# kevaday/alphazero-general

Measured on AMD Instinct MI355X. Metric: mcts_node_expansions_per_sec, higher is better.
Workload: dtype f32 tree / f16 net; 1 GPU; connect4 self-play, 2048 games/GPU x 100 sims/move, fp16 ResNet 128ch x 8, random-init, noise+temp on; games_per_gpu=2048, sims_per_move=100, hipgraph_rounds=True, stream_pipelines=1, fused_search_launch=True, mfma_tower=True, ranks=1

## Files before the change

alphazero_general_amd/build.py:

```python
import os
import subprocess
import sys

HERE = os.path.dirname(os.path.abspath(__file__))
SRC = os.path.join(HERE, 'csrc', 'azg_engine.hip')
DEPS = [os.path.join(HERE, 'csrc', f) for f in sorted(os.listdir(os.path.join(HERE, 'csrc')))] + \
       [os.path.join(os.path.dirname(HERE), 'include', 'azg.h')]
OUT = os.path.join(HERE, 'lib', 'libazg_hip.so')
FLAGS = ['--offload-arch=gfx950', '-O3', '-std=c++17', '-ffp-contract=off', '-fPIC', '-shared']
VARIANTS = {
    'product': ('libazg_hip.so', []),
    'debug': ('libazg_debug.so', ['-DAZG_DEBUG_BOUNDS']),
    'tuning': ('libazg_tuning.so', ['-DAZG_TUNING']),
    'timing-tree': ('libazg_timing.so', ['-DAZG_TREE_TIMING']),
    'timing-tower': ('libazg_timing.so', ['-DAZG_TOWER_TIMING']),
    'timing-w1': ('libazg_timing_w1.so', ['-DAZG_TOWER_TIMING', '-DAZG_PHASE_TID=64', '-DAZG_TUNING']),
    'timing-w1-overlap': ('libazg_timing_w1o.so', ['-DAZG_TOWER_TIMING', '-DAZG_PHASE_TID=64', '-DAZG_OVL_NW=2', '-DHEADS_A_RING=1', '-DAZG_TUNING']),
    'ring1': ('libazg_ring1.so', ['-DHEADS_A_RING=1', '-DAZG_TUNING']),
    'overlap': ('libazg_overlap.so', ['-DAZG_OVL_NW=2', '-DHEADS_A_RING=1', '-DAZG_TUNING']),
    'headline1': ('libazg_headline1.so', ['-DAZG_HEADLINE_ONE_WG']),
}


def hipcc():
    for c in (os.environ.get('HIPCC'), '/opt/rocm/bin/hipcc', 'hipcc'):
        if c and (os.path.isabs(c) and os.path.exists(c) or not os.path.isabs(c)):
            return c
    return 'hipcc'


def source_sha(variant='product'):
    import hashlib
    h = hashlib.sha256()
    for f in DEPS:
# ... 34 lines not shown
```

alphazero_general_amd/csrc/azg_conv.h:

```cpp
#pragma once
#include <hip/hip_runtime.h>
#include <stdint.h>
#include <type_traits>

namespace azg {

typedef _Float16 half8 __attribute__((ext_vector_type(8)));
typedef _Float16 half4 __attribute__((ext_vector_type(4)));
typedef float floatx4 __attribute__((ext_vector_type(4)));

struct TowerParams {
    const void *x;
    const void *w;
    const float *bias;
    const float *pre_scale;
    const float *pre_shift;
    void *y;
    int boards, nblocks;
    const void *head_w;
    const float *head_b;
    float *policy, *value;
    int A, NV;
    unsigned long long *dbg;
    const void *head1_w;
    const float *head1_b;
// ... 535 lines not shown
    if constexpr (__is_same(SEARCH, NoSearch)) return 0; else return sa.ev.gcount[GC_ERROR];
}
template <class SEARCH, class = void> struct WideGameOf { using type = C4; };
template <class SEARCH> struct WideGameOf<SEARCH, std::void_t<typename SEARCH::Game>> { using type = typename SEARCH::Game; };
#ifdef AZG_HEADLINE_ONE_WG
#define AZG_SEARCH_MIN_BLOCKS 1
#else
#define AZG_SEARCH_MIN_BLOCKS 2
#endif
template <class SEARCH> constexpr int tower_min_blocks() { if constexpr (__is_same(SEARCH, NoSearch)) return 2; else { if constexpr (SEARCH::WIDE) return SEARCH::MIN_BLOCKS; else return AZG_SEARCH_MIN_BLOCKS; } }

template <int H, int W, int C> constexpr bool tower_khalf_order() { return ((H == 7 && W == 7) || (H == 8 && W == 8)) && C == 64; }
template <int C, int BOARDS> constexpr int tower_layer_param_bytes(int nblocks) { return ((2 * nblocks + 1) * C * 4 + 2 * nblocks * C * 2 + C * 4 + 15) / 16 * 16; }
template <int C, int BOARDS, bool SOLO = false> constexpr int tower_param_bytes(int nblocks) {
    return BOARDS == 1 ? tower_layer_param_bytes<C, BOARDS>(nblocks) + (C / 32) * 2 * 1024 + 128 : SOLO ? tower_layer_param_bytes<C, BOARDS>(nblocks) : 0;
}
template <int H, int W, int BOARDS, int C, int PSPLIT = 1, class SEARCH = NoSearch, int KSPLIT = 1>
__global__ __launch_bounds__(C * 2 * PSPLIT * KSPLIT, tower_min_blocks<SEARCH>()) void k_tower2(TowerParams Pin, const int16_t *pixmap, SEARCH sa) {
    using GEO = TowerGeom<H, W, BOARDS, C>;
    constexpr bool IS_SEARCH = !__is_same(SEARCH, NoSearch);
    constexpr bool IS_WIDE = []() { if constexpr (IS_SEARCH) return SEARCH::WIDE; else return false; }();
    static_assert(!IS_SEARCH || IS_WIDE || (PSPLIT == 1 && C == 128 && BOARDS <= C / 32), "search mode: one wave per game, fused heads");
    constexpr bool IS_ARENA = []() { if constexpr (IS_SEARCH) { if constexpr (!SEARCH::WIDE) return SEARCH::ARENA; } return false; }();
    static_assert(!IS_ARENA || BOARDS == 1, "arena search: one game (one mover, one model) per workgroup");
    constexpr bool IS_WARENA = []() { if constexpr (IS_SEARCH) { if constexpr (SEARCH::WIDE) return SEARCH::ARENA; } return false; }();
    static_assert(!IS_WARENA || BOARDS == 1, "wide arena search: one game (one mover, one model) per workgroup");
    static_assert(!IS_WIDE || (C / 32) * PSPLIT * KSPLIT >= BOARDS, "wide search mode: at least one wavefront per game");
    constexpr bool SOLO = IS_WIDE && wide_solo<C, PSPLIT, KSPLIT, BOARDS>();
    constexpr bool EXACT = []() { if constexpr (IS_WIDE) return SEARCH::EXACT; else return false; }();
    constexpr bool HSTREAM = HeadsStreamedOf<SEARCH, H * W, C>::value;
// ... 124 lines not shown
        if constexpr (IS_SEARCH) nsims = sa.sims + (IS_WIDE ? 1 : 0);
        [[maybe_unused]] const int sc_off = PARAM_OFF + (2 * P.nblocks + 1) * C * 4, sh_off = sc_off + P.nblocks * C * 2;
        [[maybe_unused]] const int h1_off = PARAM_OFF + tower_layer_param_bytes<C, BOARDS>(P.nblocks);
        if (PLDS && !raw) {
            float *pb_ = reinterpret_cast<float *>(smem + PARAM_OFF);
            _Float16 *psc_ = reinterpret_cast<_Float16 *>(smem + sc_off), *psh_ = reinterpret_cast<_Float16 *>(smem + sh_off);
            for (int c = tid; c < (2 * P.nblocks + 1) * C; c += NT) pb_[c] = P.bias[c];
            for (int c = tid; c < P.nblocks * C; c += NT) { psc_[c] = (_Float16)P.pre_scale[c]; psh_[c] = (_Float16)P.pre_shift[c]; }
            if (PLDS_H1 && P.head_w == nullptr && P.head1_w != nullptr) {
                uint4 *h1_ = reinterpret_cast<uint4 *>(smem + h1_off);
                for (int c = tid; c < KS * 2 * 64; c += NT) h1_[c] = reinterpret_cast<const uint4 *>(P.head1_w)[c];
                if (tid < 32) reinterpret_cast<float *>(smem + h1_off + KS * 2 * 1024)[tid] = P.head1_b[tid];
            }
        }
        [[maybe_unused]] bool lds_live = false;
        for (int sim = 0; sim < nsims; sim++) {
        int lane_sim = lane_k;
        if constexpr (IS_WIDE) asm volatile("" : "+v"(lane_sim));
        const int lane = lane_sim, tid = wave * 64 + lane, g = lane >> 4, i16 = lane & 15;
#ifdef AZG_TOWER_TIMING
        unsigned long long wt_[6] = {0, 0, 0, 0, 0, 0};
#define AZG_WPHASE(i) do { if (IS_WIDE) wt_[i] = __builtin_amdgcn_s_memtime(); } while (0)
#else
#define AZG_WPHASE(i) do { } while (0)
#endif
        AZG_WPHASE(0);
        if constexpr (IS_WIDE) {
            using G = typename SEARCH::Game;
            using WS = WideScratch<G, HW, SOLO>;
            static_assert(G::CELLS == HW, "game / tower geometry mismatch");
// ... 208 lines not shown
                } else {
                    char *row = img + GEO::qrow(bd * HW + lane) * RS;
                    const uint4 z = make_uint4(0, 0, 0, 0);
                    *reinterpret_cast<uint4 *>(row) = z; *reinterpret_cast<uint4 *>(row + 16) = z;
                    *reinterpret_cast<uint4 *>(row + 32) = z; *reinterpret_cast<uint4 *>(row + 48) = z;
                }
            }
            if (sim == sa.sims) break;
            AZG_WPHASE(1);
            if (raw) { __syncthreads(); continue; }
        } else if constexpr (IS_SEARCH) {
            using G = typename SEARCH::Game;
            static_assert(G::CELLS == HW && G::A < 8, "search mode needs a game whose tree functions use no LDS scratch");
            if ((sim & 15) == 0) {
                int *flag = reinterpret_cast<int *>(img + SCRATCH_PV + 512);
                if (tid == 0) *flag = sa.ev.gcount[GC_ERROR];
                __syncthreads();
                const int err = *flag;
                __syncthreads();
                if (tid == 0) *flag = 0;
                if (err) break;
            }
            int slot = tile * BOARDS + wave;
            asm volatile("" : "+v"(slot));
            slot = __builtin_amdgcn_readfirstlane(slot);
            if (wave >= BOARDS) {
            } else if (slot < sa.ev.B) {
                select_slot<G>(sa.ev, slot, lane, nullptr, [&](const typename G::S &st, int ln) {
                    if (ln < HW) {
                        char *row = img + GEO::qrow(wave * HW + ln) * RS;
                        *reinterpret_cast<half8 *>(row) = G::obs8(st, ln);
                        const uint4 z = make_uint4(0, 0, 0, 0);
                        *reinterpret_cast<uint4 *>(row + 16) = z; *reinterpret_cast<uint4 *>(row + 32) = z; *reinterpret_cast<uint4 *>(row + 48) = z;
                    }
                });
            } else if (lane < HW) {
                char *row = img + GEO::qrow(wave * HW + lane) * RS;
                const uint4 z = make_uint4(0, 0, 0, 0);
                *reinterpret_cast<uint4 *>(row) = z; *reinterpret_cast<uint4 *>(row + 16) = z;
                *reinterpret_cast<uint4 *>(row + 32) = z; *reinterpret_cast<uint4 *>(row + 48) = z;
            }
        } else {
            const uint4 *xg = reinterpret_cast<const uint4 *>(P.x) + (size_t)row0;
            for (int c = tid; c < ROWS * 4; c += NT) {
                const int p = c >> 2, chunk = c & 3;
                uint4 v = make_uint4(0, 0, 0, 0);
                if (chunk == 0 && p < rows_here) v = xg[p];
                *reinterpret_cast<uint4 *>(img + GEO::qrow(p) * RS + chunk * 16) = v;
            }
        }
#ifdef AZG_TOWER_TIMING
        if (P.dbg && tid == 0) P.dbg[1024 + blockIdx.x * 2] = __builtin_amdgcn_s_memtime();
#endif
        const half8 *wt = wm0;
#pragma unroll
        for (int j = 0; j < WR - 1; j++) { const half8 *f = stream_frag<GEO, KSPLIT>(wl, wm0, j); a[j][0] = f[0]; a[j][1] = f[64]; }
#ifdef AZG_TOWER_TIMING
        asm volatile("s_waitcnt vmcnt(0)");
        if (P.dbg && tid == 0) P.dbg[1024 + blockIdx.x * 2 + 1] = __builtin_amdgcn_s_memtime();
#endif
        __syncthreads();
#ifdef AZG_TOWER_TIMING
#define AZG_STAMP2(i) do { if (P.dbg && blockIdx.x == 0 && tile == 0 && lane == 0) P.dbg[(layer * 4 + wave) * 5 + (i)] = __builtin_amdgcn_s_memtime(); } while (0)
#define AZG_WGSTAMP(i) do { if (P.dbg && tid == 0) P.dbg[2048 + (size_t)blockIdx.x * 8 + (i)] = __builtin_amdgcn_s_memtime(); } while (0)
#else
#define AZG_STAMP2(i) do { } while (0)
#define AZG_WGSTAMP(i) do { } while (0)
#endif
        AZG_WGSTAMP(4);
        [[maybe_unused]] floatx4 bnext[2];
        if constexpr (PLDS) {
#pragma unroll
            for (int m = 0; m < 2; m++) bnext[m] = *reinterpret_cast<const floatx4 *>(smem + PARAM_OFF + ((2 * cg + m) * 16 + g * 4) * 4);
        }
        for (int layer = 0; layer <= 2 * P.nblocks; layer++) {
            AZG_STAMP2(0);
            if ((layer ^ slot_role) & 1) __builtin_amdgcn_s_setprio(2); else __builtin_amdgcn_s_setprio(0);
            const float *bias = P.bias + (size_t)layer * C;
            const bool is_s = (layer & 1) == 0;
            const int nb = layer >> 1;
            const bool has_next = nb < P.nblocks;
            const half2v zero2 = {(_Float16)0.f, (_Float16)0.f};
#pragma unroll
            for (int m = 0; m < 2; m++) {
// ... 109 lines not shown
                        } else {
                            *reinterpret_cast<uint4 *>(img + off) = *reinterpret_cast<uint4 *>(v);
                        }
                    }
                }
            }
            if constexpr (PLDS) {
#pragma unroll
                for (int m = 0; m < 2; m++) bnext[m] = *reinterpret_cast<const floatx4 *>(smem + PARAM_OFF + ((layer + 1) * C + (2 * cg + m) * 16 + g * 4) * 4);
            }
            AZG_STAMP2(3);
            __syncthreads();
            AZG_STAMP2(4);
        }
        AZG_WGSTAMP(5);
        AZG_WPHASE(2);
        if (P.head_w == nullptr && P.head1_w != nullptr) {
            [[maybe_unused]] _Float16 *feat_lds = nullptr;
            if constexpr (IS_WIDE) feat_lds = reinterpret_cast<_Float16 *>(smem + TILE + WideScratch<typename SEARCH::Game, HW, SOLO>::FEAT);
            using HGame = typename std::conditional<IS_WIDE, typename WideGameOf<SEARCH>::type, C4>::type;
            [[maybe_unused]] HeadsFirst<HGame, HW, HSTREAM ? HEADS_STREAM_RING : WideScratch<HGame, HW>::FK / 32> hfirst;
            constexpr bool HEADS_EARLY = EXACT && BOARDS == 1;
            if constexpr (OVL) {
                if (wave >= 1 && wave <= OVL_NW) heads_full_prefetch<typename SEARCH::Game, HW, OVL_NW, true>(hfs, wave - 1, lane, hfirst);
                if (IS_WIDE && tid == 0 && (sim & 15) == 15) {
                    using WLE = WideLds<typename WideGameOf<SEARCH>::type, HW, BOARDS, SOLO, HSTREAM>;
                    *reinterpret_cast<int *>(smem + TILE + WLE::ERR) = sa_error_word(sa);
                }
            } else
            if constexpr (HSTREAM) { static_assert(HEADS_EARLY && !OVL, "streamed heads: the one-game exact tile"); heads_stream_prefetch<typename SEARCH::Game, HW, NT / 64>(hfs, wave, lane, hfirst); } else
// ... 108 lines not shown
                            if (!bvalid || p >= HW) bf[j][ks] = zero8;
                        }
                    }
                }
                __builtin_amdgcn_sched_barrier(0);
#pragma unroll
                for (int j = 0; j < JB; j++)
                    if (j0 + j < NPW) {
#pragma unroll
                        for (int ks = 0; ks < 4; ks++) hacc4[ks] = __builtin_amdgcn_mfma_f32_16x16x32_f16(af[j][ks], bf[j][ks], hacc4[ks], 0, 0, 0);
                    }
                __builtin_amdgcn_sched_barrier(0);
            }
            const floatx4 hacc = (hacc4[0] + hacc4[1]) + (hacc4[2] + hacc4[3]);
            AZG_WGSTAMP(6);
            __syncthreads();
            float *red = reinterpret_cast<float *>(img);
            if (wave < 4) {
#pragma unroll
                for (int r = 0; r < 4; r++) red[(wave * 16 + g * 4 + r) * 16 + i16] = hacc[r];
            }
            __syncthreads();
            const int nb_here = min(BOARDS, P.boards - tile * BOARDS);
            if (tid < 64) {
                const int bd = tid >> 4, o = tid & 15, A = P.A, NV = P.NV;
                const int bc = bd < BOARDS ? bd : 0;
                const float lgt = ((red[(0 * 16 + o) * 16 + bc] + red[(1 * 16 + o) * 16 + bc]) + (red[(2 * 16 + o) * 16 + bc] + red[(3 * 16 + o) * 16 + bc]))
                                  + P.head_b[o];
                const bool isp = o < A, isv = o >= A && o < A + NV;
                float mp = isp ? lgt : -INFINITY, mv = isv ? lgt : -INFINITY;
#pragma unroll
                for (int d = 8; d; d >>= 1) { mp = fmaxf(mp, __shfl_xor(mp, d, 16)); mv = fmaxf(mv, __shfl_xor(mv, d, 16)); }
                const float e = isp ? __expf(lgt - mp) : isv ? __expf(lgt - mv) : 0.f;
                float sp = isp ? e : 0.f, sv = isv ? e : 0.f;
#pragma unroll
                for (int d = 8; d; d >>= 1) { sp += __shfl_xor(sp, d, 16); sv += __shfl_xor(sv, d, 16); }
                if constexpr (IS_SEARCH) {
                    reinterpret_cast<float *>(img + SCRATCH_PV)[bd * 16 + o] = isp ? e / sp : e / sv;
                } else if (bd < nb_here) {
                    if (isp) P.policy[(size_t)(tile * BOARDS + bd) * A + o] = e / sp;
                    if (isv) P.value[(size_t)(tile * BOARDS + bd) * NV + (o - A)] = e / sv;
                }
            }
            if constexpr (IS_SEARCH) {
                using G = typename SEARCH::Game;
                __syncthreads();
                int slot = tile * BOARDS + wave;
                asm volatile("" : "+v"(slot));
                slot = __builtin_amdgcn_readfirstlane(slot);
                const float *pv = reinterpret_cast<const float *>(img + SCRATCH_PV) + wave * 16;
                if (wave < BOARDS && slot < sa.ev.B) backup_slot<G>(sa.ev, slot, lane, pv, pv + P.A, nullptr, nullptr);
            }
            AZG_WGSTAMP(7);
            __syncthreads();
            if (tid < 256) reinterpret_cast<uint4 *>(img)[tid] = make_uint4(0, 0, 0, 0);
            if constexpr (IS_SEARCH) { if (tid < 16) reinterpret_cast<uint4 *>(img + SCRATCH_PV)[tid] = make_uint4(0, 0, 0, 0); }
        }
        if constexpr (!OVL) __syncthreads();
        }
        if constexpr (IS_WIDE) {
            using G = typename SEARCH::Game;
            using WS = WideScratch<G, HW, SOLO>;
            __syncthreads();
            const int bd = wave % BOARDS, role = wave / BOARDS, slot = tile * BOARDS + bd;
            const int tree = IS_WARENA ? slot * sa.ev.T + (reinterpret_cast<const int *>(smem + TILE + WideLds<G, HW, BOARDS, SOLO, HSTREAM>::ERR)[1] & 15) : slot;
            if (lds_live && role == 0 && slot < sa.ev.B) {
                const char *ws = smem + TILE + bd * WS::BYTES;
                if (lane < 4) reinterpret_cast<uint4 *>(sa.ev.hdr + tree)[lane] = reinterpret_cast<const uint4 *>(ws + WS::HDR)[lane];
                static_assert(sizeof(TreeHdr) == 4 * sizeof(uint4) && sizeof(azg_state) % 16 == 0 && sizeof(PathEnt) == sizeof(uint4),
                              "the LDS mirror moves the header, the root state and the path as whole 16-byte chunks");
                if constexpr (!SOLO) {
                    const int depth = *reinterpret_cast<const int *>(ws + WS::HDR + offsetof(TreeHdr, depth));
                    for (int j = lane; j < depth && j < sa.ev.maxd; j += 64)
                        reinterpret_cast<uint4 *>(sa.ev.path + (size_t)tree * sa.ev.maxd)[j] = reinterpret_cast<const uint4 *>(ws + WS::PATH)[j];
// ... 17 lines not shown
```

alphazero_general_amd/csrc/azg_engine.hip:

```cpp
#include <hip/hip_runtime.h>
#include <hip/hip_ext.h>
#include <cstdio>
#include <cstdlib>
#include <cstring>
#include <map>
#include <mutex>
#include <string>
#include <vector>
#include "azg_kernels.h"
#include "azg_conv.h"

using namespace azg;

static thread_local std::string g_err;
static int fail(int code, const std::string &msg) { g_err = msg; return code; }
#define HIPCHK(x) do { hipError_t _e = (x); if (_e != hipSuccess) return fail(AZG_E_HIP, std::string(#x) + ": " + hipGetErrorString(_e)); } while (0)

struct EvPair { hipEvent_t a, b; bool ext; };

static thread_local EvPair *g_kev = nullptr;
#define AZG_LAUNCH(kernel, grid, block, lds, stream, ...) do { \
    if (g_kev) { hipExtLaunchKernelGGL(kernel, grid, block, lds, stream, g_kev->a, g_kev->b, 0, __VA_ARGS__); g_kev = nullptr; } \
    else hipLaunchKernelGGL(kernel, grid, block, lds, stream, __VA_ARGS__); } while (0)

// ... 778 lines not shown
    if (LDS_BYTES > (size_t)d_lds[dev]) return fail(AZG_E_INVALID_ARG, "this tower does not fit the LDS of its tile (too many residual blocks)");
    if (occ) {
        int n = 0;
        HIPCHK(hipOccupancyMaxActiveBlocksPerMultiprocessor(&n, reinterpret_cast<const void *>(&k_tower2<H, W, BOARDS, C, PSPLIT, SEARCH, KSPLIT>),
                                                            C * 2 * PSPLIT * KSPLIT, LDS_BYTES));
        *occ = n > 0 ? n : 1;
    }
    if (init_only) return AZG_OK;
    HIPCHK(hipDeviceGetAttribute(&cus, hipDeviceAttributeMultiprocessorCount, dev));
    const int ntiles = (P.boards + BOARDS - 1) / BOARDS + (P.rows_per_model ? P.nmodels - 1 : 0);
    {
        const int per_cu = (int)((size_t)d_lds[dev] / LDS_BYTES) > 0 ? (int)((size_t)d_lds[dev] / LDS_BYTES) : 1;
        const int grid = IS_SEARCH || ntiles < per_cu * cus ? ntiles : per_cu * cus;
#ifdef AZG_TOWER_TIMING
        static unsigned long long *dbg = nullptr; static int calls = 0;
        if (!dbg) { HIPCHK(hipMalloc((void **)&dbg, (2048 + 4096 * 8) * 8)); HIPCHK(hipMemset(dbg, 0, (2048 + 4096 * 8) * 8)); }
        TowerParams Q = P; Q.dbg = dbg;
        AZG_LAUNCH((k_tower2<H, W, BOARDS, C, PSPLIT, SEARCH, KSPLIT>), dim3(grid), dim3(C * 2 * PSPLIT * KSPLIT), LDS_BYTES, s, Q, (const int16_t *)d_map[dev], sa);
        if constexpr (IS_SEARCH) if constexpr (SEARCH::WIDE) {
            static unsigned long long w[512 * 4];
            HIPCHK(hipStreamSynchronize(s)); HIPCHK(hipMemcpy(w, dbg + 2048 + 4096 * 4, sizeof(unsigned long long) * 4 * (grid < 512 ? grid : 512), hipMemcpyDeviceToHost));
            double ph[4] = {0, 0, 0, 0}; const int nb = grid < 512 ? grid : 512;
            for (int b = 0; b < nb; b++) for (int i = 0; i < 4; i++) ph[i] += (double)w[b * 4 + i];
            const double n = (double)nb * (sa.sims > 8 ? sa.sims - 8 : 1);
            fprintf(stderr, "wide search, cycles per simulation (mean over %d workgroups): tree %.0f tower %.0f headconv %.0f heads %.0f\n", nb, ph[0] / n, ph[1] / n, ph[2] / n, ph[3] / n);
            HIPCHK(hipMemset(dbg + 2048 + 4096 * 4, 0, sizeof(unsigned long long) * 4 * 512));
            static unsigned long long hw_[512 * 8];
            HIPCHK(hipMemcpy(hw_, dbg + 2048 + 4096 * 5, sizeof(unsigned long long) * 8 * nb, hipMemcpyDeviceToHost));
            double hp[5] = {0, 0, 0, 0, 0}, hn = 0;
            for (int b = 0; b < nb; b++) { for (int i = 0; i < 5; i++) hp[i] += (double)hw_[b * 8 + i]; hn += (double)hw_[b * 8 + 5]; }
            if (hn > 0) fprintf(stderr, "  helper wavefront (cycles per simulation with a policy backup): header %.0f masks %.0f logits %.0f softmax %.0f priors %.0f\n",
                                hp[0] / hn, hp[1] / hn, hp[2] / hn, hp[3] / hn, hp[4] / hn);
            HIPCHK(hipMemset(dbg + 2048 + 4096 * 5, 0, sizeof(unsigned long long) * 8 * 512));
            {
                unsigned long long h[64 * 4 * 5];
                HIPCHK(hipMemcpy(h, dbg, sizeof(h), hipMemcpyDeviceToHost));
                for (int l = 0; l <= 2 * P.nblocks; l++) for (int w = 0; w < C / 32 * PSPLIT * KSPLIT && w < 4; w++) {
                    unsigned long long *t = h + (l * 4 + w) * 5;
                    fprintf(stderr, "  layer %2d wave %d: main %6llu wait %6llu epi %6llu bar %6llu | start %llu\n", l, w, t[1] - t[0], t[2] - t[1], t[3] - t[2], t[4] - t[3], t[0] - h[0]);
                }
            }
            calls = 100;
        }
        if (++calls == 8) {
            unsigned long long h[64 * 4 * 5];
            HIPCHK(hipStreamSynchronize(s)); HIPCHK(hipMemcpy(h, dbg, sizeof(h), hipMemcpyDeviceToHost));
            for (int l = 0; l <= 2 * P.nblocks; l++) for (int w = 0; w < C / 32; w++) {
                unsigned long long *t = h + (l * 4 + w) * 5;
                fprintf(stderr, "layer %2d wave %d: main %6llu wait %6llu epi %6llu bar %6llu | start %llu\n", l, w, t[1] - t[0], t[2] - t[1], t[3] - t[2], t[4] - t[3], t[0] - h[0]);
            }
            static unsigned long long w[4096 * 8];
            HIPCHK(hipMemcpy(w, dbg + 2048, sizeof(unsigned long long) * 8 * grid, hipMemcpyDeviceToHost));
            unsigned long long x2[1024];
            HIPCHK(hipMemcpy(x2, dbg + 1024, sizeof(x2), hipMemcpyDeviceToHost));
            for (int b = 0; b < grid && b < 512; b++) fprintf(stderr, "wgx %4d xload+store %llu weights %llu\n", b, x2[b * 2] - w[b * 8], x2[b * 2 + 1] - x2[b * 2]);
            for (int b = 0; b < grid; b++) fprintf(stderr, "wg %4d xcc %llu hwid %08llx start %llu end %llu | prologue %llu layers %llu headmm %llu softmax %llu tail %llu\n", b, w[b * 8 + 3] & 15, w[b * 8 + 2], w[b * 8], w[b * 8 + 1],
                                                   w[b * 8 + 4] - w[b * 8], w[b * 8 + 5] - w[b * 8 + 4], w[b * 8 + 6] - w[b * 8 + 5], w[b * 8 + 7] - w[b * 8 + 6], w[b * 8 + 1] - w[b * 8 + 7]);
        }
// ... 195 lines not shown
    return r;
}

extern "C" int azg_search_f16(azg_engine *e, void *stream, const void *w, const float *bias, const float *pre_scale, const float *pre_shift,
                              int nblocks, const void *head_w, const float *head_b, int sims) {
    if (!e || !w || !bias || !head_w || !head_b || nblocks < 0 || sims < 0) return fail(AZG_E_INVALID_ARG, "null or out-of-range argument");
    if (nblocks > 0 && (!pre_scale || !pre_shift)) return fail(AZG_E_INVALID_ARG, "pre_scale/pre_shift required");
    if (e->cfg.game != AZG_GAME_CONNECT4 || e->v.arena)
        return fail(AZG_E_UNSUPPORTED, "the fused search kernel is built for connect4 self-play with a 128-channel tower (use azg_select / network / azg_backup)");
    const int A = e->gi.action_size, NV = e->gi.num_players + 1;
    TowerParams P{nullptr, w, bias, pre_scale, pre_shift, nullptr, e->v.B, nblocks, head_w, head_b, nullptr, nullptr, A, NV, nullptr, nullptr, nullptr, nullptr, 0, nullptr, 0, {}};
    SearchArgs<C4> sa{e->v, sims};
    EvPair ep; const bool prof = sims > 0 && netprof_begin((hipStream_t)stream, ep);
    int r, cus = 1;
    r = device_cus(&cus); if (r != AZG_OK) { g_kev = nullptr; return r; }
    if (2 * e->v.B <= 5 * cus) r = launch_tower<C4::H, C4::W, 1, 128, 1, SearchArgs<C4>>((hipStream_t)stream, P, sa, sims == 0);
    else if (e->v.B <= 5 * cus) r = launch_tower<C4::H, C4::W, 2, 128, 1, SearchArgs<C4>>((hipStream_t)stream, P, sa, sims == 0);
    else r = launch_tower<C4::H, C4::W, 4, 128, 1, SearchArgs<C4>>((hipStream_t)stream, P, sa, sims == 0);
    netprof_end((hipStream_t)stream, 2, prof, ep);
    return r;
}

extern "C" int azg_search_arena_f16(azg_engine *e, void *stream, int nmodels, const void *const *w, const float *const *bias, const float *const *pre_scale,
                                    const float *const *pre_shift, int nblocks, const void *const *head_w, const float *const *head_b,
                                    const int32_t *p2i_host, const uint32_t *seat_of_slot, int sims) {
    if (!e || !w || !bias || !head_w || !head_b || nblocks < 0 || sims < 0 || (!p2i_host && !seat_of_slot)) return fail(AZG_E_INVALID_ARG, "null or out-of-range argument");
    if (e->cfg.game != AZG_GAME_CONNECT4 || !e->v.arena)
        return fail(AZG_E_UNSUPPORTED, "the persistent arena launch is built for connect4 arena engines with 128-channel towers (use azg_select / network / azg_backup)");
    if (nmodels < 1 || nmodels > 4 || nmodels < e->gi.num_players) return fail(AZG_E_UNSUPPORTED, "one model per player, at most 4");
    for (int m = 0; m < nmodels; m++)
        if (!w[m] || !bias[m] || !head_w[m] || !head_b[m] || (nblocks > 0 && (!pre_scale || !pre_shift || !pre_scale[m] || !pre_shift[m]))) return fail(AZG_E_INVALID_ARG, "null model parameter");
    const int A = e->gi.action_size, NV = e->gi.num_players + 1;
// ... 397 lines not shown
```

alphazero_general_amd/csrc/azg_kernels.h:

```cpp
#pragma once
#include "azg_games.h"

namespace azg {

struct NodeR {
    int n; float q, p, v; int fc; int a, nchild, player, e;
};
AZG_DEV void unpack(const uint4 &lo, const uint4 &hi, NodeR &r) {
    r.n = (int)lo.x; r.q = __uint_as_float(lo.y); r.p = __uint_as_float(lo.z); r.v = __uint_as_float(lo.w);
    r.fc = (int)hi.x; r.a = hi.y & 0xFFFF; r.nchild = hi.y >> 16; r.player = hi.z & 0xFF; r.e = (hi.z >> 8) & 0xFF;
}
AZG_DEV uint4 pack_hi(int fc, int a, int nchild, int player, int e) {
    return make_uint4((unsigned)fc, (unsigned)(a & 0xFFFF) | ((unsigned)nchild << 16), (unsigned)player | ((unsigned)e << 8), 0u);
}
AZG_DEV void load_node(const Node *p, uint4 &lo, uint4 &hi) {
    const uint4 *q = reinterpret_cast<const uint4 *>(p);
    lo = q[0]; hi = q[1];
}
AZG_DEV void raise_error(const View &ev, int code) { atomicCAS(&ev.gcount[GC_ERROR], 0, code); }
#ifdef AZG_DEBUG_BOUNDS
AZG_DEV bool bounds_fail(const View &ev, int site) { raise_error(ev, AZG_E_INTERNAL); atomicCAS(&ev.gcount[GC_BOUNDS_SITE], 0, site); return false; }
#define AZG_BOUNDS_OK(ev, site, cond) ((cond) ? true : bounds_fail(ev, site))
#else
#define AZG_BOUNDS_OK(ev, site, cond) true
// ... 323 lines not shown
        for (int a = 0; a < A; a++) {
            uint64_t bal = __ballot(ca[0] == a);
            if (bal) s += rl(cp[0], __ffsll((unsigned long long)bal) - 1);
        }
        return s;
    } else {
        if (first) { for (int a = lane; a < A; a += 64) m_lds[a] = 0.f; }
        wave_sync();
#pragma unroll
        for (int c = 0; c < NC; c++) if (ca[c] >= 0) m_lds[ca[c]] = cp[c];
        wave_sync();
        return np_sum_static<A>(m_lds, scr, lane);
    }
}

template <class G, int NC>
AZG_DEV void leaf_policy(const View &ev, int slot, Node *nodes, int fc, int k, bool at_root, const float *pi, float *m_lds, float *scr, int lane) {
    int ca[NC]; float cp[NC];
#pragma unroll
    for (int c = 0; c < NC; c++) {
        int i = c * 64 + lane;
        ca[c] = i < k ? (int)nodes[fc + i].a : -1;
        cp[c] = i < k ? pi[ca[c]] : 0.f;
    }
    const float s = masked_sum<G, NC>(ev, ca, cp, m_lds, scr, lane, true);
    if (!(s > 0.f) && lane == 0) raise_error(ev, AZG_E_FLOATING_POINT);
#pragma unroll
    for (int c = 0; c < NC; c++) cp[c] = cp[c] / s;
    if (at_root && ev.add_temp) {
        const double ex = 1.0 / (double)ev.root_temp;
#pragma unroll
        for (int c = 0; c < NC; c++) cp[c] = np_pow_f32(cp[c], ex);
        const float s2 = masked_sum<G, NC>(ev, ca, cp, m_lds, scr, lane, false);
#pragma unroll
        for (int c = 0; c < NC; c++) cp[c] = cp[c] / s2;
    }
    if (at_root && ev.add_noise) {
        const uint64_t ctr = ev.tape_ctr[slot];
// ... 18 lines not shown
            const double inv = 1.0 / acc;
#pragma unroll
            for (int c = 0; c < NC; c++) nzv[c] = (float)(g[c] * inv);
        }
#pragma unroll
        for (int c = 0; c < NC; c++) {
            const float nz = nzv[c];
            cp[c] = (float)(((double)cp[c] * (1.0 - (double)ev.noise_frac)) + (double)(ev.noise_frac * nz));
        }
        if (lane == 0) ev.tape_ctr[slot] = ctr + 1;
    }
#pragma unroll
    for (int c = 0; c < NC; c++) { int i = c * 64 + lane; if (i < k) nodes[fc + i].p = cp[c]; }
}

template <class G>
AZG_DEV void backup_policy(const View &ev, int slot, const HdrR &hr, Node *nodes, const float *pi, float *m_lds, float *scr, int lane) {
    constexpr int NCH = (G::MAXK + 63) / 64;
    if (hr.leaf_e || hr.leaf_fc < 0) return;
    const int k = hr.leaf_k, fc = hr.leaf_fc;
    if (!AZG_BLOCK_OK(ev, 4, fc, k, hr.alloc)) return;
    const bool at_root = hr.leaf == LEAF_IS_ROOT;
    if constexpr (NCH > 1) {
        if (k > 64) leaf_policy<G, NCH>(ev, slot, nodes, fc, k, at_root, pi, m_lds, scr, lane);
        else leaf_policy<G, 1>(ev, slot, nodes, fc, k, at_root, pi, m_lds, scr, lane);
    } else leaf_policy<G, 1>(ev, slot, nodes, fc, k, at_root, pi, m_lds, scr, lane);
}

template <class G>
AZG_DEV void backup_path(const View &ev, int slot, int tree, HdrR &hr, Node *nodes, const float (&vrow)[G::P + 1], int lane) {
    constexpr int P = G::P, NV = P + 1, NE = P + G::HAS_DRAW;
    TreeHdr *h = ev.hdr + tree;
// ... 43 lines not shown
}

template <class G>
AZG_DEV void backup_slot(const View &ev, int slot, int lane, const float *pi, const float *vrow, float *m_lds, float *scr) {
    const int tree = tree_of_slot(ev, slot);
    HdrR hr; load_hdr(ev.hdr + tree, hr);
    Node *nodes = tree_nodes(ev, tree, hr.base);
    float val[G::P + 1];
#pragma unroll
    for (int j = 0; j < G::P + 1; j++) val[j] = hr.leaf_e ? 0.f : vrow[j];
    AZG_TSTAMP(ev, slot, lane, 1);
    backup_policy<G>(ev, slot, hr, nodes, pi, m_lds, scr, lane);
    AZG_TSTAMP(ev, slot, lane, 2);
    backup_path<G>(ev, slot, tree, hr, nodes, val, lane);
    AZG_TSTAMP(ev, slot, lane, 3);
}

template <class G>
__global__ __launch_bounds__(64) void k_backup(View ev, const float *policy, const float *value, const int32_t *row_of_slot) {
    if (__builtin_amdgcn_readfirstlane(ev.gcount[GC_ERROR]) != 0) return;
    __shared__ float m_lds[G::A < 8 ? 8 : G::A];
    __shared__ float scr[64];
    const int slot = blockIdx.x;
    const int row = row_of_slot ? row_of_slot[slot] : slot;
    backup_slot<G>(ev, slot, threadIdx.x, policy + (size_t)row * G::A, value + (size_t)row * (G::P + 1), m_lds, scr);
}

AZG_DEV void flag_set_gen(int *f, int gen, int lane) { if (lane == 0) __hip_atomic_store(f, gen, __ATOMIC_RELEASE, __HIP_MEMORY_SCOPE_WORKGROUP); }
AZG_DEV void flag_wait_gen(const View &ev, int *f, int gen) {
    for (int spin = 0; spin < (1 << 23); spin++) {
// ... 561 lines not shown
```

Before: 7.961 million expansions/s.

## Move search backup into per-wave lanes and drop per-sim workgroup barriers

In the non-wide search tower, each wave now reduces its own head logits and does the softmax in registers. It feeds the backup directly from lane shuffles (PiLanes) instead of staging policy/value through LDS scratch, which removes several __syncthreads per simulation. The error-flag check now runs only at sim 0, with waves OR-ing errors into the flag every 16 sims. An optional AZG_FUSED_WALK path fuses backup with the next selection, but it is off by default. Tail timing instrumentation and an AZG_SEARCH_BOARDS tuning override are also added. The risk is cross-wave LDS hazards now that barriers are removed.

```diff
diff --git a/alphazero_general_amd/build.py b/alphazero_general_amd/build.py
--- a/alphazero_general_amd/build.py
+++ b/alphazero_general_amd/build.py
@@ -18,6 +18,7 @@
     'timing-w1-overlap': ('libazg_timing_w1o.so', ['-DAZG_TOWER_TIMING', '-DAZG_PHASE_TID=64', '-DAZG_OVL_NW=2', '-DHEADS_A_RING=1', '-DAZG_TUNING']),
     'ring1': ('libazg_ring1.so', ['-DHEADS_A_RING=1', '-DAZG_TUNING']),
     'overlap': ('libazg_overlap.so', ['-DAZG_OVL_NW=2', '-DHEADS_A_RING=1', '-DAZG_TUNING']),
+    'fusedwalk': ('libazg_fusedwalk.so', ['-DAZG_FUSED_WALK=1']),
     'headline1': ('libazg_headline1.so', ['-DAZG_HEADLINE_ONE_WG']),
 }
 
diff --git a/alphazero_general_amd/csrc/azg_conv.h b/alphazero_general_amd/csrc/azg_conv.h
--- a/alphazero_general_amd/csrc/azg_conv.h
+++ b/alphazero_general_amd/csrc/azg_conv.h
@@ -9,6 +9,10 @@
 typedef _Float16 half4 __attribute__((ext_vector_type(4)));
 typedef float floatx4 __attribute__((ext_vector_type(4)));
 
+#ifndef AZG_FUSED_WALK
+#define AZG_FUSED_WALK 0
+#endif
+#define AZG_TAIL_OFF (2048 + 4096 * 8)
 struct TowerParams {
     const void *x;
     const void *w;
@@ -574,6 +578,24 @@
 template <int C, int BOARDS> constexpr int tower_layer_param_bytes(int nblocks) { return ((2 * nblocks + 1) * C * 4 + 2 * nblocks * C * 2 + C * 4 + 15) / 16 * 16; }
 template <int C, int BOARDS, bool SOLO = false> constexpr int tower_param_bytes(int nblocks) {
     return BOARDS == 1 ? tower_layer_param_bytes<C, BOARDS>(nblocks) + (C / 32) * 2 * 1024 + 128 : SOLO ? tower_layer_param_bytes<C, BOARDS>(nblocks) : 0;
+}
+template <class G, class GEO>
+__device__ __forceinline__ void search_leaf_rows(char *img, int bd, const typename G::S &st, int ln) {
+    if (ln < GEO::HW) {
+        char *row = img + GEO::qrow(bd * GEO::HW + ln) * GEO::RSTRIDE;
+        *reinterpret_cast<half8 *>(row) = G::obs8(st, ln);
+        const uint4 z = make_uint4(0, 0, 0, 0);
+        *reinterpret_cast<uint4 *>(row + 16) = z; *reinterpret_cast<uint4 *>(row + 32) = z; *reinterpret_cast<uint4 *>(row + 48) = z;
+    }
+}
+template <class GEO>
+__device__ __forceinline__ void search_zero_rows(char *img, int bd, int lane) {
+    if (lane < GEO::HW) {
+        char *row = img + GEO::qrow(bd * GEO::HW + lane) * GEO::RSTRIDE;
+        const uint4 z = make_uint4(0, 0, 0, 0);
+        *reinterpret_cast<uint4 *>(row) = z; *reinterpret_cast<uint4 *>(row + 16) = z;
+        *reinterpret_cast<uint4 *>(row + 32) = z; *reinterpret_cast<uint4 *>(row + 48) = z;
+    }
 }
 template <int H, int W, int BOARDS, int C, int PSPLIT = 1, class SEARCH = NoSearch, int KSPLIT = 1>
 __global__ __launch_bounds__(C * 2 * PSPLIT * KSPLIT, tower_min_blocks<SEARCH>()) void k_tower2(TowerParams Pin, const int16_t *pixmap, SEARCH sa) {
@@ -728,6 +750,13 @@
             }
         }
         [[maybe_unused]] bool lds_live = false;
+#ifdef AZG_TOWER_TIMING
+        [[maybe_unused]] unsigned tl_acc[8] = {0, 0, 0, 0, 0, 0, 0, 0}, tl_n = 0;
+        [[maybe_unused]] unsigned long long tl_prev = __builtin_amdgcn_s_memtime();
+#define AZG_TAIL(i) do { if constexpr (IS_SEARCH && !IS_WIDE) { const unsigned long long t_ = __builtin_amdgcn_s_memtime(); tl_acc[i] += (unsigned)(t_ - tl_prev); tl_prev = t_; } } while (0)
+#else
+#define AZG_TAIL(i) do { } while (0)
+#endif
         for (int sim = 0; sim < nsims; sim++) {
         int lane_sim = lane_k;
         if constexpr (IS_WIDE) asm volatile("" : "+v"(lane_sim));
@@ -966,31 +995,25 @@
             static_assert(G::CELLS == HW && G::A < 8, "search mode needs a game whose tree functions use no LDS scratch");
             if ((sim & 15) == 0) {
                 int *flag = reinterpret_cast<int *>(img + SCRATCH_PV + 512);
-                if (tid == 0) *flag = sa.ev.gcount[GC_ERROR];
-                __syncthreads();
+                if (sim == 0) {
+                    if (tid == 0) *flag = sa.ev.gcount[GC_ERROR];
+                    __syncthreads();
+                }
                 const int err = *flag;
-                __syncthreads();
-                if (tid == 0) *flag = 0;
                 if (err) break;
             }
-            int slot = tile * BOARDS + wave;
-            asm volatile("" : "+v"(slot));
-            slot = __builtin_amdgcn_readfirstlane(slot);
-            if (wave >= BOARDS) {
-            } else if (slot < sa.ev.B) {
-                select_slot<G>(sa.ev, slot, lane, nullptr, [&](const typename G::S &st, int ln) {
-                    if (ln < HW) {
-                        char *row = img + GEO::qrow(wave * HW + ln) * RS;
-                        *reinterpret_cast<half8 *>(row) = G::obs8(st, ln);
-                        const uint4 z = make_uint4(0, 0, 0, 0);
-                        *reinterpret_cast<uint4 *>(row + 16) = z; *reinterpret_cast<uint4 *>(row + 32) = z; *reinterpret_cast<uint4 *>(row + 48) = z;
-                    }
-                });
-            } else if (lane < HW) {
-                char *row = img + GEO::qrow(wave * HW + lane) * RS;
-                const uint4 z = make_uint4(0, 0, 0, 0);
-                *reinterpret_cast<uint4 *>(row) = z; *reinterpret_cast<uint4 *>(row + 16) = z;
-                *reinterpret_cast<uint4 *>(row + 32) = z; *reinterpret_cast<uint4 *>(row + 48) = z;
+            AZG_TAIL(5);
+            if (!AZG_FUSED_WALK || (sim & 15) == 0) {
+                int slot = tile * BOARDS + wave;
+                asm volatile("" : "+v"(slot));
+                slot = __builtin_amdgcn_readfirstlane(slot);
+                if (wave >= BOARDS) {
+                } else if (slot < sa.ev.B) {
+                    select_slot<G>(sa.ev, slot, lane, nullptr, [&](const typename G::S &st, int ln) { search_leaf_rows<G, GEO>(img, wave, st, ln); });
+                } else {
+                    search_zero_rows<GEO>(img, wave, lane);
+                }
+                AZG_TAIL(6);
             }
         } else {
             const uint4 *xg = reinterpret_cast<const uint4 *>(P.x) + (size_t)row0;
@@ -1020,6 +1043,7 @@
 #define AZG_WGSTAMP(i) do { } while (0)
 #endif
         AZG_WGSTAMP(4);
+        AZG_TAIL(7);
         [[maybe_unused]] floatx4 bnext[2];
         if constexpr (PLDS) {
 #pragma unroll
@@ -1159,6 +1183,7 @@
             AZG_STAMP2(4);
         }
         AZG_WGSTAMP(5);
+        AZG_TAIL(0);
         AZG_WPHASE(2);
         if (P.head_w == nullptr && P.head1_w != nullptr) {
             [[maybe_unused]] _Float16 *feat_lds = nullptr;
@@ -1297,13 +1322,52 @@
             }
             const floatx4 hacc = (hacc4[0] + hacc4[1]) + (hacc4[2] + hacc4[3]);
             AZG_WGSTAMP(6);
+            AZG_TAIL(1);
             __syncthreads();
             float *red = reinterpret_cast<float *>(img);
-            if (wave < 4) {
+            if (wave < 4 && (!(IS_SEARCH && !IS_WIDE) || i16 < BOARDS)) {
 #pragma unroll
                 for (int r = 0; r < 4; r++) red[(wave * 16 + g * 4 + r) * 16 + i16] = hacc[r];
             }
             __syncthreads();
+            if constexpr (IS_SEARCH && !IS_WIDE) {
+                using G = typename SEARCH::Game;
+                int slot = tile * BOARDS + wave;
+                asm volatile("" : "+v"(slot));
+                slot = __builtin_amdgcn_readfirstlane(slot);
+                const bool look_next = ((sim + 1) & 15) == 0, more = sim + 1 < nsims, fuse = AZG_FUSED_WALK && more && !look_next;
+                if (wave < BOARDS) {
+                    const int o = i16, A = P.A, NV = P.NV;
+                    float *c0 = &red[(0 * 16 + o) * 16 + wave], *c1 = &red[(1 * 16 + o) * 16 + wave], *c2 = &red[(2 * 16 + o) * 16 + wave], *c3 = &red[(3 * 16 + o) * 16 + wave];
+                    const float lgt = ((*c0 + *c1) + (*c2 + *c3)) + P.head_b[o];
+                    if (lane < 16) { *c0 = 0.f; *c1 = 0.f; *c2 = 0.f; *c3 = 0.f; }
+                    const bool isp = o < A, isv = o >= A && o < A + NV;
+                    float mp = isp ? lgt : -INFINITY, mv = isv ? lgt : -INFINITY;
+#pragma unroll
+                    for (int d = 8; d; d >>= 1) { mp = fmaxf(mp, __shfl_xor(mp, d, 16)); mv = fmaxf(mv, __shfl_xor(mv, d, 16)); }
+                    const float e = isp ? __expf(lgt - mp) : isv ? __expf(lgt - mv) : 0.f;
+                    float sp = isp ? e : 0.f, sv = isv ? e : 0.f;
+#pragma unroll
+                    for (int d = 8; d; d >>= 1) { sp += __shfl_xor(sp, d, 16); sv += __shfl_xor(sv, d, 16); }
+                    const float prob = isp ? e / sp : e / sv;
+                    AZG_TAIL(2);
+                    if (slot < sa.ev.B) {
+                        if (fuse)
+                            backup_select_slot<G>(sa.ev, slot, lane, prob, [&](const typename G::S &st, int ln) { search_leaf_rows<G, GEO>(img, wave, st, ln); });
+                        else backup_slot_lanes<G>(sa.ev, slot, lane, prob);
+                    } else if (fuse) {
+                        search_zero_rows<GEO>(img, wave, lane);
+                    }
+                    wave_sync();
+                    if (more && look_next && lane == 0) {
+                        const int err = __hip_atomic_load(&sa.ev.gcount[GC_ERROR], __ATOMIC_RELAXED, __HIP_MEMORY_SCOPE_AGENT);
+                        if (err) atomicOr(reinterpret_cast<int *>(img + SCRATCH_PV + 512), err);
+                    }
+                } else { AZG_TAIL(2); }
+                AZG_WGSTAMP(7);
+                AZG_TAIL(3);
+                if (more && look_next) __syncthreads();
+            } else {
             const int nb_here = min(BOARDS, P.boards - tile * BOARDS);
             if (tid < 64) {
                 const int bd = tid >> 4, o = tid & 15, A = P.A, NV = P.NV;
@@ -1318,29 +1382,35 @@
                 float sp = isp ? e : 0.f, sv = isv ? e : 0.f;
 #pragma unroll
                 for (int d = 8; d; d >>= 1) { sp += __shfl_xor(sp, d, 16); sv += __shfl_xor(sv, d, 16); }
-                if constexpr (IS_SEARCH) {
-                    reinterpret_cast<float *>(img + SCRATCH_PV)[bd * 16 + o] = isp ? e / sp : e / sv;
-                } else if (bd < nb_here) {
+                if (bd < nb_here) {
                     if (isp) P.policy[(size_t)(tile * BOARDS + bd) * A + o] = e / sp;
                     if (isv) P.value[(size_t)(tile * BOARDS + bd) * NV + (o - A)] = e / sv;
                 }
-            }
-            if constexpr (IS_SEARCH) {
-                using G = typename SEARCH::Game;
-                __syncthreads();
-                int slot = tile * BOARDS + wave;
-                asm volatile("" : "+v"(slot));
-                slot = __builtin_amdgcn_readfirstlane(slot);
-                const float *pv = reinterpret_cast<const float *>(img + SCRATCH_PV) + wave * 16;
-                if (wave < BOARDS && slot < sa.ev.B) backup_slot<G>(sa.ev, slot, lane, pv, pv + P.A, nullptr, nullptr);
             }
             AZG_WGSTAMP(7);
             __syncthreads();
             if (tid < 256) reinterpret_cast<uint4 *>(img)[tid] = make_uint4(0, 0, 0, 0);
-            if constexpr (IS_SEARCH) { if (tid < 16) reinterpret_cast<uint4 *>(img + SCRATCH_PV)[tid] = make_uint4(0, 0, 0, 0); }
-        }
-        if constexpr (!OVL) __syncthreads();
-        }
+            }
+        }
+        if constexpr (!OVL && !(IS_SEARCH && !IS_WIDE)) __syncthreads();
+        AZG_TAIL(4);
+#ifdef AZG_TOWER_TIMING
+        tl_n++;
+#endif
+        }
+        if constexpr (IS_SEARCH && !IS_WIDE) {
+            __syncthreads();
+            if (tid == 0) *reinterpret_cast<int *>(img + SCRATCH_PV + 512) = 0;
+        }
+#ifdef AZG_TOWER_TIMING
+        if constexpr (IS_SEARCH && !IS_WIDE) {
+            if (P.dbg && tid == 0 && blockIdx.x < 4096) {
+                unsigned long long *d = P.dbg + AZG_TAIL_OFF + (size_t)blockIdx.x * 16;
+                for (int i = 0; i < 8; i++) d[i] = tl_acc[i];
+                d[8] = tl_n;
+            }
+        }
+#endif
         if constexpr (IS_WIDE) {
             using G = typename SEARCH::Game;
             using WS = WideScratch<G, HW, SOLO>;
diff --git a/alphazero_general_amd/csrc/azg_engine.hip b/alphazero_general_amd/csrc/azg_engine.hip
--- a/alphazero_general_amd/csrc/azg_engine.hip
+++ b/alphazero_general_amd/csrc/azg_engine.hip
@@ -1,5 +1,6 @@
 #include <hip/hip_runtime.h>
 #include <hip/hip_ext.h>
+#include <algorithm>
 #include <cstdio>
 #include <cstdlib>
 #include <cstring>
@@ -816,7 +817,7 @@
         const int grid = IS_SEARCH || ntiles < per_cu * cus ? ntiles : per_cu * cus;
 #ifdef AZG_TOWER_TIMING
         static unsigned long long *dbg = nullptr; static int calls = 0;
-        if (!dbg) { HIPCHK(hipMalloc((void **)&dbg, (2048 + 4096 * 8) * 8)); HIPCHK(hipMemset(dbg, 0, (2048 + 4096 * 8) * 8)); }
+        if (!dbg) { HIPCHK(hipMalloc((void **)&dbg, (AZG_TAIL_OFF + 4096 * 16) * 8)); HIPCHK(hipMemset(dbg, 0, (AZG_TAIL_OFF + 4096 * 16) * 8)); }
         TowerParams Q = P; Q.dbg = dbg;
         AZG_LAUNCH((k_tower2<H, W, BOARDS, C, PSPLIT, SEARCH, KSPLIT>), dim3(grid), dim3(C * 2 * PSPLIT * KSPLIT), LDS_BYTES, s, Q, (const int16_t *)d_map[dev], sa);
         if constexpr (IS_SEARCH) if constexpr (SEARCH::WIDE) {
@@ -844,6 +845,32 @@
             }
             calls = 100;
         }
+        if constexpr (IS_SEARCH) if constexpr (!SEARCH::WIDE) {
+            hipStreamCaptureStatus cap = hipStreamCaptureStatusNone;
+            HIPCHK(hipStreamIsCapturing(s, &cap));
+            if (cap == hipStreamCaptureStatusNone && sa.sims > 0) {
+                static unsigned long long t[4096 * 16];
+                static const char *names[10] = {"tower", "head_gemm", "head_reduce_softmax", "backup", "zero_barriers", "error_look", "select", "ring_wait", "period", "tail_share_ppm"};
+                const int nb = grid < 4096 ? grid : 4096;
+                HIPCHK(hipStreamSynchronize(s)); HIPCHK(hipMemcpy(t, dbg + AZG_TAIL_OFF, sizeof(unsigned long long) * 16 * nb, hipMemcpyDeviceToHost));
+                std::vector<double> col[10];
+                for (int b = 0; b < nb; b++) {
+                    const double n = (double)t[b * 16 + 8];
+                    if (n <= 0) continue;
+                    double per = 0;
+                    for (int i = 0; i < 8; i++) { col[i].push_back((double)t[b * 16 + i] / n); per += (double)t[b * 16 + i] / n; }
+                    col[8].push_back(per); col[9].push_back(per > 0 ? 1e6 * (per - (double)t[b * 16] / n) / per : 0);
+                }
+                fprintf(stderr, "headline-tail launch: games_per_workgroup %d workgroups %d sims %d\n", BOARDS, (int)col[0].size(), sa.sims);
+                for (int i = 0; i < 10 && !col[0].empty(); i++) {
+                    std::sort(col[i].begin(), col[i].end());
+                    const size_t m = col[i].size();
+                    fprintf(stderr, "headline-tail %s median %.0f p10 %.0f p90 %.0f min %.0f max %.0f\n", names[i], col[i][m / 2], col[i][m / 10], col[i][m * 9 / 10], col[i][0], col[i][m - 1]);
+                }
+                HIPCHK(hipMemset(dbg + AZG_TAIL_OFF, 0, sizeof(unsigned long long) * 16 * 4096));
+                calls = 100;
+            }
+        }
         if (++calls == 8) {
             unsigned long long h[64 * 4 * 5];
             HIPCHK(hipStreamSynchronize(s)); HIPCHK(hipMemcpy(h, dbg, sizeof(h), hipMemcpyDeviceToHost));
@@ -1069,8 +1096,14 @@
     EvPair ep; const bool prof = sims > 0 && netprof_begin((hipStream_t)stream, ep);
     int r, cus = 1;
     r = device_cus(&cus); if (r != AZG_OK) { g_kev = nullptr; return r; }
-    if (2 * e->v.B <= 5 * cus) r = launch_tower<C4::H, C4::W, 1, 128, 1, SearchArgs<C4>>((hipStream_t)stream, P, sa, sims == 0);
-    else if (e->v.B <= 5 * cus) r = launch_tower<C4::H, C4::W, 2, 128, 1, SearchArgs<C4>>((hipStream_t)stream, P, sa, sims == 0);
+#ifdef AZG_TUNING
+    static const int forced = getenv("AZG_SEARCH_BOARDS") ? atoi(getenv("AZG_SEARCH_BOARDS")) : 0;
+#else
+    constexpr int forced = 0;
+#endif
+    const int bt = forced ? forced : 2 * e->v.B <= 5 * cus ? 1 : e->v.B <= 5 * cus ? 2 : 4;
+    if (bt == 1) r = launch_tower<C4::H, C4::W, 1, 128, 1, SearchArgs<C4>>((hipStream_t)stream, P, sa, sims == 0);
+    else if (bt == 2) r = launch_tower<C4::H, C4::W, 2, 128, 1, SearchArgs<C4>>((hipStream_t)stream, P, sa, sims == 0);
     else r = launch_tower<C4::H, C4::W, 4, 128, 1, SearchArgs<C4>>((hipStream_t)stream, P, sa, sims == 0);
     netprof_end((hipStream_t)stream, 2, prof, ep);
     return r;
diff --git a/alphazero_general_amd/csrc/azg_kernels.h b/alphazero_general_amd/csrc/azg_kernels.h
--- a/alphazero_general_amd/csrc/azg_kernels.h
+++ b/alphazero_general_amd/csrc/azg_kernels.h
@@ -361,14 +361,18 @@
     }
 }
 
-template <class G, int NC>
-AZG_DEV void leaf_policy(const View &ev, int slot, Node *nodes, int fc, int k, bool at_root, const float *pi, float *m_lds, float *scr, int lane) {
+AZG_DEV float pi_child(const float *pi, int a, bool on) { return on ? pi[a] : 0.f; }
+struct PiLanes { float x; };
+AZG_DEV float pi_child(const PiLanes &pi, int a, bool on) { const float v = __shfl(pi.x, a & 15); return on ? v : 0.f; }
+
+template <class G, int NC, class PI>
+AZG_DEV void leaf_policy(const View &ev, int slot, Node *nodes, int fc, int k, bool at_root, const PI &pi, float *m_lds, float *scr, int lane) {
     int ca[NC]; float cp[NC];
 #pragma unroll
     for (int c = 0; c < NC; c++) {
         int i = c * 64 + lane;
         ca[c] = i < k ? (int)nodes[fc + i].a : -1;
-        cp[c] = i < k ? pi[ca[c]] : 0.f;
+        cp[c] = pi_child(pi, ca[c], i < k);
     }
     const float s = masked_sum<G, NC>(ev, ca, cp, m_lds, scr, lane, true);
     if (!(s > 0.f) && lane == 0) raise_error(ev, AZG_E_FLOATING_POINT);
@@ -417,8 +421,8 @@
     for (int c = 0; c < NC; c++) { int i = c * 64 + lane; if (i < k) nodes[fc + i].p = cp[c]; }
 }
 
-template <class G>
-AZG_DEV void backup_policy(const View &ev, int slot, const HdrR &hr, Node *nodes, const float *pi, float *m_lds, float *scr, int lane) {
+template <class G, class PI>
+AZG_DEV void backup_policy(const View &ev, int slot, const HdrR &hr, Node *nodes, const PI &pi, float *m_lds, float *scr, int lane) {
     constexpr int NCH = (G::MAXK + 63) / 64;
     if (hr.leaf_e || hr.leaf_fc < 0) return;
     const int k = hr.leaf_k, fc = hr.leaf_fc;
@@ -492,6 +496,35 @@
     AZG_TSTAMP(ev, slot, lane, 2);
     backup_path<G>(ev, slot, tree, hr, nodes, val, lane);
     AZG_TSTAMP(ev, slot, lane, 3);
+}
+
+template <class G>
+AZG_DEV void backup_slot_lanes(const View &ev, int slot, int lane, float prob) {
+    static_assert(G::A < 8 && G::A + G::P + 1 <= 16, "a row of at most 16 outputs, no LDS scratch");
+    const int tree = tree_of_slot(ev, slot);
+    HdrR hr; load_hdr(ev.hdr + tree, hr);
+    Node *nodes = tree_nodes(ev, tree, hr.base);
+    float val[G::P + 1];
+#pragma unroll
+    for (int j = 0; j < G::P + 1; j++) { const float v = __shfl(prob, G::A + j); val[j] = hr.leaf_e ? 0.f : v; }
+    backup_policy<G>(ev, slot, hr, nodes, PiLanes{prob}, nullptr, nullptr, lane);
+    backup_path<G>(ev, slot, tree, hr, nodes, val, lane);
+}
+
+template <class G, class Sink>
+AZG_DEV void backup_select_slot(const View &ev, int slot, int lane, float prob, Sink &&sink) {
+    static_assert(G::A < 8 && G::A + G::P + 1 <= 16, "a row of at most 16 outputs, no LDS scratch");
+    const int tree = tree_of_slot(ev, slot);
+    HdrR hr; load_hdr(ev.hdr + tree, hr);
+    Node *nodes = tree_nodes(ev, tree, hr.base);
+    float val[G::P + 1];
+#pragma unroll
+    for (int j = 0; j < G::P + 1; j++) { const float v = __shfl(prob, G::A + j); val[j] = hr.leaf_e ? 0.f : v; }
+    backup_policy<G>(ev, slot, hr, nodes, PiLanes{prob}, nullptr, nullptr, lane);
+    backup_path<G>(ev, slot, tree, hr, nodes, val, lane);
+    wave_sync();
+    const uint64_t ctr = ev.tape_ctr[slot];
+    select_tree<G>(ev, slot, tree, hr, G::load(&ev.states[slot], lane), ctr, lane, nullptr, sink, NoGate{}, NoRanks{});
 }
 
 template <class G>
```

New measurement: 7.956 million expansions/s. About the same (-0.1%).
